# IML-DKFZ/values

Hardware: AMD Instinct MI355X
Metric: uncertainty-volumes/sec (64^3, T=10 MC-dropout) (higher is better)
Workload: dtype f32; 1 GPU; C2: 64^3 1-channel volumes, UNet3D(initial_filter_size=8, 2 classes), T=10 MC-dropout passes + fused softmax/entropy/MI/variance/argmax reduction; dropout=hash bit generator, new seed every step, weights=torch default init, seed 123

## Files before the change

### include/values_amd.h

```cpp
#ifndef VALUES_AMD_H
#define VALUES_AMD_H

#include <stddef.h>
#include <stdint.h>

#ifdef __cplusplus
extern "C" {
#endif

typedef void* vx_stream_t;

enum {
  VX_OK = 0,
  VX_E_NULL = -1,
  VX_E_SHAPE = -2,
  VX_E_DTYPE = -3,
  VX_E_WORKSPACE = -4,
  VX_E_ALIGN = -5
};

enum { VX_F32 = 0, VX_F64 = 1 };
enum { VX_ACT_NONE = 0, VX_ACT_LRELU = 1 , VX_ACT_RELU = 2 };
enum { VX_DROP_NONE = 0, VX_DROP_HASH = 1, VX_DROP_MASK = 2 };

// ... 72 lines not shown
  const int32_t* head_dst;
  const int32_t* head_flip;
  int32_t head_C;
  const float* in_mean; const float* in_rstd;
  int32_t in_drop_mode; uint32_t in_drop_seed, in_drop_layer;
  int32_t in_repeat;
  int32_t out_xblk, out_half;
  uint32_t* range_flag;
  const uint32_t* seed_dev;
  const float* up_in;
  const float* up_w;
  const float* up_b;
  int32_t up_pitch;
  float* pool_out;
  uint32_t* pool_flags;
  int32_t in_split;
  int32_t out_f16, in_f16;
  int32_t out_split, up_split;
  const float* up_fused;
  const uint32_t* in_pool_flags;
  const float* acc_in;
  int32_t acc_pitch;
  int32_t out_planar, in_planar;
  int32_t products;
} vx_conv3d_args;
int64_t vx_conv3d_upfused_packed_floats(void);
int vx_pack_conv3d_upfused(const float* w1_torch, const float* b1, const float* up_w_torch, const float* up_b, float* packed,
                           vx_stream_t stream);
int vx_conv3d_k3_prologue_ok(int D, int H, int W, int Cin, int Cout);
int vx_conv3d_k3_upfuse_ok(int D, int H, int W, int Cin, int Cout);
int64_t vx_convT_zc16_packed_floats(void);
int vx_pack_convT_zc16(const float* w_torch , float* packed, vx_stream_t stream);
int vx_conv3d_k3_skip_prologue_ok(int D, int H, int W, int Cin, int Cout, int xblk);
int vx_conv3d_k3_acc_ok(int D, int H, int W, int Cin, int Cout);
int vx_conv3d_k3_planar_ok(int D, int H, int W, int Cin, int Cout);
int vx_conv3d_k3_poolfuse_ok(int D, int H, int W, int Cin, int Cout);
int vx_conv3d_k3_presplit_ok(int D, int H, int W, int Cin, int Cout);
int vx_conv3d_k3_poolfin_ok(int Cin, int Cout);
int vx_prenorm_split(float* x, const float* mean, const float* rstd, int N, int64_t nvox, float scale, vx_stream_t stream);
int vx_pool_finish(const float* pool_raw, const uint32_t* pool_flags, const float* mean, const float* rstd, float* out,
                   int out_pitch, int N, int64_t voxels_per_sample, int drop_scale2, vx_stream_t stream);
int vx_pool_finish_z(const float* pool_raw, const uint32_t* pool_flags, const float* mean, const float* rstd, float* out,
                     int out_pitch, int N, int Dp, int64_t plane_voxels, int drop_scale2, vx_stream_t stream);
int vx_conv3d_k3_pool_layout(int D, int H, int W, int Cin, int Cout);
int vx_conv3d_k3_tiles(int D, int H, int W);
int vx_conv3d_k3_tiles_for(int D, int H, int W, int Cout);
int vx_conv3d_k3(const vx_conv3d_args* a, vx_stream_t stream);
int vx_conv3d_k3_head_fusable(int Cin, int Cout);

int vx_conv3d_k3_c1_tiles(int D, int H, int W);
int vx_conv3d_k3_c1(const float* in, const float* w_torch , const float* bias, float* out,
                    int out_pitch, int N, int D, int H, int W, int Cout, int repeat, const int32_t* src,
                    const int32_t* flip, float* stats_partial, vx_stream_t stream);

int vx_pack_input_cl8(const float* in, float* out, int N, int Cin, int D, int H, int W, int repeat, const int32_t* src,
                      const int32_t* flip, vx_stream_t stream);

int vx_instnorm_finalize(const float* stats_partial, int N, int ntiles, int C, int64_t nvox, float eps,
                         float* mean, float* rstd, vx_stream_t stream);

typedef struct vx_norm_args {
  const float* x; int32_t x_pitch;
  const float* mean; const float* rstd;
  float* out; int32_t out_pitch, out_coff;
  float* pool_out; int32_t pool_pitch;
  int32_t N, D, H, W, C;
  int32_t act, drop_mode; uint32_t drop_seed, drop_layer; const uint8_t* drop_mask;
  int32_t out_xblk, out_half;
  int32_t x_xblk, x_half;
  const uint32_t* seed_dev;
  uint32_t* range_flag;
} vx_norm_args;
int vx_norm_act_drop_pool(const vx_norm_args* a, vx_stream_t stream);
typedef struct vx_stat_src {
  const float* stats_partial; int32_t tiles; float eps; int64_t count;
  float* mean_out; float* rstd_out;
} vx_stat_src;
int vx_norm_act_drop_pool_stats(const vx_norm_args* a, const vx_stat_src* st, vx_stream_t stream);
int vx_prenorm_split_stats(float* x, const vx_stat_src* st, int N, int64_t nvox, float scale, vx_stream_t stream);
int vx_zero(void* p, int64_t bytes, vx_stream_t stream);
int vx_pool_finish_z_stats(const float* pool_raw, const uint32_t* pool_flags, const vx_stat_src* st, float* out, int out_pitch,
                           int N, int Dp, int64_t plane_voxels, int drop_scale2, vx_stream_t stream);
int vx_norm_act_drop_pool_bcast(const vx_norm_args* a, int x_repeat, vx_stream_t stream);

typedef struct vx_convT_args {
  const float* in; int32_t in_pitch;
  const float* w_packed; const float* bias;
  float* out; int32_t out_pitch, out_coff;
  int32_t N, D, H, W, Cin, Cout;
  int32_t act, drop_mode; uint32_t drop_seed, drop_layer; const uint8_t* drop_mask;
  int32_t out_xblk, out_half;
  uint32_t* range_flag;
  const uint32_t* seed_dev;
} vx_convT_args;
int vx_convT_k2s2(const vx_convT_args* a, vx_stream_t stream);

int vx_conv1x1_ncdhw(const float* in, int in_pitch, const float* w, const float* bias, float* out, int N, int D,
                     int H, int W, int F, int C, const int32_t* dst, const int32_t* flip, vx_stream_t stream);

typedef struct vx_unet3d_weights {
  const float* conv_w[18];
  const float* conv_b[18];
  const float* up_w[4];
  const float* up_b[4];
  const float* final_w;
  const float* final_b;
// ... 221 lines not shown
```

### values_amd/_lib.py

```python
from __future__ import annotations

import ctypes as C
import os

_HERE = os.path.dirname(os.path.abspath(__file__))
LIB_PATH = os.environ.get("VX_LIB_PATH") or os.path.join(_HERE, "libvalues_amd.so")

VX_F32, VX_F64 = 0, 1
VX_ACT_NONE, VX_ACT_LRELU, VX_ACT_RELU = 0, 1, 2
VX_DROP_NONE, VX_DROP_HASH, VX_DROP_MASK = 0, 1, 2

_p = C.c_void_p
_i = C.c_int
_i32 = C.c_int32
_u32 = C.c_uint32
_i64 = C.c_int64


class ConvArgs(C.Structure):
    _fields_ = [("in_", _p), ("w_packed", _p), ("bias", _p), ("out", _p),
                ("in_pitch", _i32), ("out_pitch", _i32), ("out_coff", _i32),
                ("N", _i32), ("D", _i32), ("H", _i32), ("W", _i32), ("Cin", _i32), ("Cout", _i32),
                ("act", _i32), ("drop_mode", _i32), ("drop_seed", _u32), ("drop_layer", _u32),
                ("drop_mask", _p), ("stats_partial", _p), ("in_xblk", _i32), ("w_family", _i32),
# ... 116 lines not shown
                  "distance beyond the output start", "output capacity reached", "checksum mismatch", "ISIZE mismatch",
                  "trailing bytes", "stored block length mismatch", "preset dictionary")
VX_INFLATE_CAPACITY = 7


class NiftiDecItem(C.Structure):
    _fields_ = [("src", _p), ("src_n", _i64), ("vox_offset", _i64), ("dst", _p), ("dst_n", _i64), ("ndim", _i32),
                ("dims", _i32 * 7), ("code", _i32), ("big_endian", _i32), ("out_dtype", _i32), ("pad", _i32),
                ("slope", C.c_double), ("inter", C.c_double)]


SIGNATURES = {
    "vx_version": (_i, []),
    "vx_last_error_string": (C.c_char_p, []),
    "vx_last_kernel_name": (C.c_char_p, []),
    "vx_drop_hash_mask": (_i, [_u32, _u32, _i, _i64, _p, _p]),
    "vx_get_config": (_i, [C.POINTER(Config)]),
    "vx_set_config": (_i, [C.POINTER(Config)]),
    "vx_conv3d_k3_family": (_i, [_i, _i]),
    "vx_conv2d_family": (_i, [_i, _i, _i]),
    "vx_unc_reduce": (_i, [_p, _i, _i, _i, _i, _i, _i64, _p, _p, _p, _p, _p, _p, _p]),
    "vx_unc_reduce_ex": (_i, [_p, _i, _i, _i, _i, _i, _i64, C.POINTER(UncOutputs), _p]),
    "vx_unc_stats_accumulate": (_i, [_p, _i, _i, _i, _i64, _p, _p]),
    "vx_unc_stats_finalize": (_i, [_p, _i, _i, _i, _i64, _p, _p, _p, _p, _p, _p]),
    "vx_softmax_planar": (_i, [_p, _i64, _i, _i64, _p, _p]),
    "vx_one_minus_msr": (_i, [_p, _i, _i, _i64, _p, _p]),
    "vx_conv3d_k3_packed_floats": (_i64, [_i, _i]),
    "vx_pack_conv3d_k3": (_i, [_p, _p, _i, _i, _p]),
    "vx_convT_k2s2_packed_floats": (_i64, [_i, _i]),
    "vx_pack_convT_k2s2": (_i, [_p, _p, _i, _i, _p]),
    "vx_conv3d_k3_tiles": (_i, [_i, _i, _i]),
    "vx_conv3d_k3_tiles_for": (_i, [_i, _i, _i, _i]),
    "vx_conv3d_k3_head_fusable": (_i, [_i, _i]),
    "vx_conv3d_k3_prologue_ok": (_i, [_i, _i, _i, _i, _i]),
    "vx_conv3d_k3_upfuse_ok": (_i, [_i, _i, _i, _i, _i]),
    "vx_conv3d_k3_poolfuse_ok": (_i, [_i, _i, _i, _i, _i]),
    "vx_conv3d_k3_presplit_ok": (_i, [_i, _i, _i, _i, _i]),
    "vx_conv3d_k3_poolfin_ok": (_i, [_i, _i]),
    "vx_conv3d_upfused_packed_floats": (_i64, []),
    "vx_pack_conv3d_upfused": (_i, [_p, _p, _p, _p, _p, _p]),
    "vx_pool_finish": (_i, [_p, _p, _p, _p, _p, _i, _i, _i64, _i, _p]),
    "vx_pool_finish_z": (_i, [_p, _p, _p, _p, _p, _i, _i, _i, _i64, _i, _p]),
    "vx_conv3d_k3_pool_layout": (_i, [_i, _i, _i, _i, _i]),
    "vx_conv3d_k3_skip_prologue_ok": (_i, [_i, _i, _i, _i, _i, _i]),
    "vx_conv3d_k3_acc_ok": (_i, [_i, _i, _i, _i, _i]),
    "vx_conv3d_k3_planar_ok": (_i, [_i, _i, _i, _i, _i]),
    "vx_convT_zc16_packed_floats": (_i64, []),
    "vx_pack_convT_zc16": (_i, [_p, _p, _p]),
    "vx_prenorm_split": (_i, [_p, _p, _p, _i, _i64, C.c_float, _p]),
    "vx_zero": (_i, [_p, _i64, _p]),
    "vx_conv3d_k3": (_i, [C.POINTER(ConvArgs), _p]),
    "vx_conv3d_k3_c1_tiles": (_i, [_i, _i, _i]),
    "vx_conv3d_k3_c1": (_i, [_p, _p, _p, _p, _i, _i, _i, _i, _i, _i, _i, _p, _p, _p, _p]),
    "vx_pack_input_cl8": (_i, [_p, _p, _i, _i, _i, _i, _i, _i, _p, _p, _p]),
    "vx_instnorm_finalize": (_i, [_p, _i, _i, _i, _i64, C.c_float, _p, _p, _p]),
    "vx_norm_act_drop_pool": (_i, [C.POINTER(NormArgs), _p]),
    "vx_norm_act_drop_pool_bcast": (_i, [C.POINTER(NormArgs), _i, _p]),
    "vx_norm_act_drop_pool_stats": (_i, [C.POINTER(NormArgs), C.POINTER(StatSrc), _p]),
    "vx_prenorm_split_stats": (_i, [_p, C.POINTER(StatSrc), _i, _i64, C.c_float, _p]),
    "vx_pool_finish_z_stats": (_i, [_p, _p, C.POINTER(StatSrc), _p, _i, _i, _i, _i64, _i, _p]),
    "vx_convT_k2s2": (_i, [C.POINTER(ConvTArgs), _p]),
    "vx_conv1x1_ncdhw": (_i, [_p, _i, _p, _p, _p, _i, _i, _i, _i, _i, _i, _p, _p, _p]),
    "vx_unet3d_workspace_bytes": (C.c_size_t, [_i, _i, _i, _i, _i]),
    "vx_unet3d_forward": (_i, [C.POINTER(UNet3DWeights), C.POINTER(UNet3DRun), _p]),
    "vx_unet3d_forward_profiled": (_i, [C.POINTER(UNet3DWeights), C.POINTER(UNet3DRun), _p, _i, C.POINTER(C.c_float),
                                        C.POINTER(C.c_char_p), C.POINTER(_i)]),
    "vx_softmax_accumulate": (_i, [_p, _i, _i, _i, _i, _i, _i, _p, _p, _p, _i, _i, _i, _i, _p]),
    "vx_aleatoric_sample": (_i, [_p, _p, _u32, _i, _i, _i, _i64, _p, _p, _p]),
    "vx_colorize_u8": (_i, [_p, _p, _i64, _p, _i, _p, _p]),
    "vx_fuse_sum": (_i, [C.POINTER(FuseArgs), _p]),
    "vx_tta_views_2d": (_i, [_p, _i, _p, _p, C.POINTER(C.c_float), C.POINTER(C.c_float), C.c_float, _i, _i, _i, _i,
                             C.POINTER(C.c_int32), _p, _p]),
    "vx_select_workspace_bytes": (_i64, []),
    "vx_select_kth": (_i, [_p, _i64, _i64, _p, _p, _p]),
    "vx_count_nonzero_u8": (_i, [_p, _i64, _p, _p]),
    "vx_mask_agreement": (_i, [_p, _i, _i, _i64, _p, _p]),
    "vx_soft_metric_workspace_bytes": (_i64, [_i, _i]),
    "vx_soft_metric_sums": (_i, [_p, _p, _i, _i, _i64, _p, _p, _p]),
    "vx_ssn2d_lowres": (_i, [_p, _i, _p, _i, _p, _u32, _i, _i64, _i, _i, _i, _p, _p, _p]),
    "vx_ssn2d_add_diag": (_i, [_p, _p, _p, _u32, _i, _i, _i64, C.c_float, _p]),
    "vx_softmax_variance": (_i, [_p, _i, _i, _i, _i, _i64, _p, _p]),
    "vx_ssn_sample": (_i, [_p, _p, _p, _u32, _i, _i, _i, _i, _i64, C.c_float, _p, _p]),
    "vx_conv2d_packed_floats": (_i64, [_i, _i, _i]),
    "vx_pack_conv2d": (_i, [_p, _p, _i, _i, _i, _p]),
    "vx_conv2d_tiles": (_i, [_i, _i, _i, _i]),
    "vx_conv2d": (_i, [C.POINTER(Conv2dArgs), _p]),
    "vx_bn_finalize": (_i, [_p, _i, _i, _i64, C.c_float, _p, _p, _p, _p, _p]),
    "vx_bn_finalize_groups": (_i, [_p, _i, _i, _i, _i, _i64, C.c_float, _p, _p, _p, _p, _p]),
    "vx_affine_gather": (_i, [C.POINTER(AffineArgs), _p]),
    "vx_bilinear_nchw": (_i, [_p, _i, _i, _i, _i, _i, _i, _i, _p, _p, _p, _p]),
    "vx_bilinear_softmax_nchw": (_i, [_p, _i, _i, _i, _i, _i, _i, _i, _p, _p, _p, _p]),
    "vx_evalmetrics_workspace_bytes": (_i64, []),
    "vx_ncc_sums": (_i, [_p, _i, _p, _i, _i64, _i, C.c_double, C.c_double, _p, _p, _p]),
    "vx_platt_sums": (_i, [_p, _i, _p, _p, _i, _i64, _i, C.c_double, C.c_double, C.c_double, C.c_double, _p, _p, _p]),
    "vx_calib_bins": (_i, [_p, _i, _p, _p, _i, _i64, _i, C.c_double, C.c_double, C.POINTER(C.c_double), _p, _p, _p]),
    "vx_box_max": (_i, [_p, _i, _i, _i, _i, _i, _i, _p, _p, _p, C.c_size_t, _p]),
    "vx_sum_thr": (_i, [_p, _i, _i64, C.c_double, _p, _p]),
    "vx_nifti_workspace_bytes": (C.c_size_t, [_i]),
    "vx_nifti_payload_bytes": (_i64, [C.POINTER(NiftiItem)]),
    "vx_nifti_payload": (_i, [C.POINTER(NiftiItem), _i, _p, _i64, _p, C.c_size_t, _p]),
    "vx_gzip_bound": (_i64, [_i64]),
    "vx_gzip_workspace_bytes": (C.c_size_t, [C.POINTER(_i64), _i]),
    "vx_gzip_encode": (_i, [C.POINTER(GzItem), _i, _p, _i64, _p, _p, C.c_size_t, _p]),
    "vx_crc32": (_i, [_p, _i64, _p, _p]),
    "vx_png_bound": (_i64, [_i, _i]),
    "vx_png_workspace_bytes": (C.c_size_t, [C.POINTER(PngItem), _i]),
# ... 91 lines not shown
```

### values_amd/csrc/conv3d_c1.hip

```cpp
#include "s16_common.h"

template <int COUT>
__global__ __launch_bounds__(256) void conv3d_k3_c1_kernel(const float* __restrict__ in, const float* __restrict__ w,
                                                           const float* __restrict__ bias,
                                                           float* __restrict__ out, int out_pitch, int N, int D, int H, int W,
                                                           int repeat, const int32_t* __restrict__ src,
                                                           const int32_t* __restrict__ flip, float* __restrict__ stats_partial,
                                                           int tiles_x, int tiles_y, int tiles_z) {
  constexpr int TX = 64, TY = 4, TZ = 4;
  constexpr int HX = TX + 2, HY = TY + 2, HZ = TZ + 2;
  __shared__ float s_in[HZ * HY * HX];
  __shared__ __attribute__((aligned(16))) float s_w[27 * COUT];
  __shared__ float s_red[16][COUT][2];

  const int tid = threadIdx.x;
  int t = blockIdx.x;
  const int tx = t % tiles_x; t /= tiles_x;
  const int ty = t % tiles_y; t /= tiles_y;
  const int tz = t % tiles_z; t /= tiles_z;
  const int n = t;
  const int v = src ? src[n] : n / repeat;
  const int f = flip ? flip[n] : 0;
  const int x0 = tx * TX, y0 = ty * TY, z0 = tz * TZ;
  const float* in_v = in + (size_t)v * D * H * W;

  for (int idx = tid; idx < HZ * HY * HX; idx += 256) {
    const int hx = idx % HX, hy = (idx / HX) % HY, hz = idx / (HX * HY);
    int gx = x0 + hx - 1, gy = y0 + hy - 1, gz = z0 + hz - 1;
    float val = 0.f;
    if ((unsigned)gx < (unsigned)W && (unsigned)gy < (unsigned)H && (unsigned)gz < (unsigned)D) {
      if (f & 1) gz = D - 1 - gz;
      if (f & 2) gy = H - 1 - gy;
      if (f & 4) gx = W - 1 - gx;
      val = in_v[((size_t)gz * H + gy) * W + gx];
    }
    s_in[idx] = val;
  }
  for (int idx = tid; idx < 27 * COUT; idx += 256) {
    const int co = idx % COUT, tap = idx / COUT;
    s_w[idx] = w[co * 27 + tap];
  }
  __syncthreads();

  const int lx = tid % TX, ly = tid / TX;
  float acc[TZ][COUT];
#pragma unroll
  for (int z = 0; z < TZ; ++z)
#pragma unroll
    for (int c = 0; c < COUT; ++c) acc[z][c] = bias[c];
#pragma unroll 1
  for (int kk = 0; kk < 9; ++kk) {
    const int ky = kk / 3, kx = kk - 3 * ky;
    float wk[3][COUT];
#pragma unroll
    for (int kz = 0; kz < 3; ++kz)
#pragma unroll
      for (int c = 0; c < COUT; c += 4) {
        const f32x4 w4 = *reinterpret_cast<const f32x4*>(&s_w[(kz * 9 + kk) * COUT + c]);
        wk[kz][c] = w4[0]; wk[kz][c + 1] = w4[1]; wk[kz][c + 2] = w4[2]; wk[kz][c + 3] = w4[3];
      }
    const float* sp = s_in + (ly + ky) * HX + lx + kx;
#pragma unroll
    for (int p = 0; p < HZ; ++p) {
      const float xv = sp[p * HY * HX];
#pragma unroll
      for (int z = 0; z < TZ; ++z) {
        const int kz = p - z;
        if (kz < 0 || kz > 2) continue;
#pragma unroll
        for (int c = 0; c < COUT; ++c) acc[z][c] = fmaf(wk[kz][c], xv, acc[z][c]);
      }
    }
  }

  const int gx = x0 + lx, gy = y0 + ly;
  float ssum[COUT], ssq[COUT];
#pragma unroll
  for (int c = 0; c < COUT; ++c) { ssum[c] = 0.f; ssq[c] = 0.f; }
#pragma unroll
  for (int z = 0; z < TZ; ++z) {
    const int gz = z0 + z;
    const bool valid = gx < W && gy < H && gz < D;
    if (valid) {
      float* o = out + (((size_t)(n * D + gz) * H + gy) * W + gx) * out_pitch;
#pragma unroll
      for (int c = 0; c < COUT; c += 4)
        *reinterpret_cast<f32x4*>(o + c) = (f32x4){acc[z][c], acc[z][c + 1], acc[z][c + 2], acc[z][c + 3]};
#pragma unroll
      for (int c = 0; c < COUT; ++c) { ssum[c] += acc[z][c]; ssq[c] = fmaf(acc[z][c], acc[z][c], ssq[c]); }
    }
  }
  if (stats_partial) {
    const int lane = tid & 63, wave = tid >> 6;
#pragma unroll
    for (int c = 0; c < COUT; ++c) {
      float s = ssum[c], q = ssq[c];
#pragma unroll
      for (int rot = 8; rot >= 1; rot >>= 1) { s += vx_row_ror(s, rot); q += vx_row_ror(q, rot); }
      if ((lane & 15) == 0) { s_red[wave * 4 + (lane >> 4)][c][0] = s; s_red[wave * 4 + (lane >> 4)][c][1] = q; }
    }
    __syncthreads();
    if (tid < COUT) {
      float s = 0.f, q = 0.f;
#pragma unroll
      for (int wv = 0; wv < 16; ++wv) { s += s_red[wv][tid][0]; q += s_red[wv][tid][1]; }
      const int ntiles = tiles_x * tiles_y * tiles_z;
      const int tile = blockIdx.x % ntiles;
      float* dst = stats_partial + (((size_t)n * ntiles + tile) * COUT + tid) * 2;
      dst[0] = s;
      dst[1] = q;
    }
  }
}

extern "C" int vx_conv3d_k3_c1_tiles(int D, int H, int W) { return ((W + 63) / 64) * ((H + 3) / 4) * ((D + 3) / 4); }

extern "C" int vx_conv3d_k3_c1(const float* in, const float* w_torch, const float* bias, float* out, int out_pitch,
                               int N, int D, int H, int W, int Cout, int repeat, const int32_t* src,
                               const int32_t* flip, float* stats_partial, vx_stream_t stream) {
  if (!in || !w_torch || !bias || !out) VX_FAIL(VX_E_NULL, "vx_conv3d_k3_c1: null pointer");
  if (N <= 0 || D <= 0 || H <= 0 || W <= 0) VX_FAIL(VX_E_SHAPE, "vx_conv3d_k3_c1: empty tensor");
  if (repeat <= 0) VX_FAIL(VX_E_SHAPE, "vx_conv3d_k3_c1: repeat must be >= 1");
  if (out_pitch < Cout || out_pitch % 4 || !vx_aligned16(out)) VX_FAIL(VX_E_ALIGN, "vx_conv3d_k3_c1: out pitch/alignment");
  const int tiles_x = (W + 63) / 64, tiles_y = (H + 3) / 4, tiles_z = (D + 3) / 4;
  dim3 grid((unsigned)(tiles_x * tiles_y * tiles_z * N));
  hipStream_t s = (hipStream_t)stream;
#define VX_C1(CO)                                                                                                  \
  vx_note_kernel("conv3d_k3_c1_kernel<" #CO ">");                                                                  \
  hipLaunchKernelGGL(conv3d_k3_c1_kernel<CO>, grid, dim3(256), 0, s, in, w_torch, bias, out, out_pitch, N, D, H, W, \
                     repeat, src, flip, stats_partial, tiles_x, tiles_y, tiles_z)
  switch (Cout) {
    case 8: VX_C1(8); break;
    case 16: VX_C1(16); break;
    case 32: VX_C1(32); break;
    default: VX_FAIL(VX_E_SHAPE, "vx_conv3d_k3_c1: Cout=%d unsupported (8, 16, 32)", Cout);
  }
#undef VX_C1
  VX_CHECK_LAUNCH("vx_conv3d_k3_c1");
  return VX_OK;
}

__global__ __launch_bounds__(256) void pack_input_cl8_kernel(const float* __restrict__ in, float* __restrict__ out, int N, int Cin,
                                                             int D, int H, int W, int repeat, const int32_t* __restrict__ src,
                                                             const int32_t* __restrict__ flip) {
  const int64_t nvox = (int64_t)D * H * W, total = (int64_t)N * nvox;
  for (int64_t i = blockIdx.x * (int64_t)blockDim.x + threadIdx.x; i < total; i += (int64_t)gridDim.x * blockDim.x) {
    const int n = (int)(i / nvox);
    const int64_t v = i - (int64_t)n * nvox;
    int x = (int)(v % W), y = (int)((v / W) % H), z = (int)(v / ((int64_t)W * H));
    const int vol = src ? src[n] : n / repeat;
    const int fl = flip ? flip[n] : 0;
    if (fl & 1) z = D - 1 - z;
    if (fl & 2) y = H - 1 - y;
    if (fl & 4) x = W - 1 - x;
    const float* p = in + ((size_t)vol * Cin) * nvox + ((size_t)z * H + y) * W + x;
    f32x4 lo = {0.f, 0.f, 0.f, 0.f}, hi = {0.f, 0.f, 0.f, 0.f};
#pragma unroll
    for (int c = 0; c < 4; ++c) {
      if (c < Cin) lo[c] = p[(size_t)c * nvox];
      if (c + 4 < Cin) hi[c] = p[(size_t)(c + 4) * nvox];
    }
    reinterpret_cast<f32x4*>(out + (size_t)i * 8)[0] = lo;
    reinterpret_cast<f32x4*>(out + (size_t)i * 8)[1] = hi;
  }
}

extern "C" int vx_pack_input_cl8(const float* in, float* out, int N, int Cin, int D, int H, int W, int repeat,
                                 const int32_t* src, const int32_t* flip, vx_stream_t stream) {
  if (!in || !out) VX_FAIL(VX_E_NULL, "vx_pack_input_cl8: null pointer");
  if (N <= 0 || D <= 0 || H <= 0 || W <= 0 || repeat <= 0) VX_FAIL(VX_E_SHAPE, "vx_pack_input_cl8: empty tensor");
  if (Cin < 1 || Cin > 8) VX_FAIL(VX_E_SHAPE, "vx_pack_input_cl8: in_channels %d (1 .. 8)", Cin);
  if (!vx_aligned16(out)) VX_FAIL(VX_E_ALIGN, "vx_pack_input_cl8: output alignment");
  const int64_t total = (int64_t)N * D * H * W;
  int bx = (int)((total + 255) / 256);
  if (bx > 16384) bx = 16384;
  vx_note_kernel("pack_input_cl8_kernel");
  hipLaunchKernelGGL(pack_input_cl8_kernel, dim3(bx), dim3(256), 0, (hipStream_t)stream, in, out, N, Cin, D, H, W, repeat, src, flip);
  VX_CHECK_LAUNCH("vx_pack_input_cl8");
  return VX_OK;
}
```

### values_amd/csrc/lib.cpp

```cpp
#include <stdarg.h>
#include <stdio.h>
#include <stdlib.h>
#include <string.h>

#include "../../include/values_amd.h"

static thread_local char g_err[512] = "";

void vx_set_error(const char* fmt, ...) {
  va_list ap;
  va_start(ap, fmt);
  vsnprintf(g_err, sizeof(g_err), fmt, ap);
  va_end(ap);
}

static thread_local const char* g_last_kernel = nullptr;
void vx_note_kernel(const char* name) { g_last_kernel = name; }
const char* vx_last_kernel() { return g_last_kernel; }
const char* vx_kname(const char* fmt, ...) {
  char buf[256];
  va_list ap;
  va_start(ap, fmt);
  vsnprintf(buf, sizeof(buf), fmt, ap);
  va_end(ap);
// ... 6 lines not shown
#include <stdlib.h>
#include <string.h>

static vx_config g_cfg;
static std::once_flag g_cfg_once;

static int env_int(const char* name, int dflt) {
  const char* e = getenv(name);
  if (!e || !*e) return dflt;
  char* end = nullptr;
  const long v = strtol(e, &end, 0);
  return end == e ? 1 : (int)v;
}

static void cfg_from_env() {
  memset(&g_cfg, 0, sizeof(g_cfg));
  g_cfg.conv_fp32 = env_int("VX_CONV_FP32", 0);
  g_cfg.s16_no_prenorm = env_int("VX_S16_NO_PRENORM", 0);
  g_cfg.s16_no_xp8 = env_int("VX_S16_NO_XP8", 0);
  g_cfg.s16_skip_raw = env_int("VX_S16_SKIP_RAW", 1);
  g_cfg.no_head_fusion = env_int("VX_NO_HEAD_FUSION", 0);
  g_cfg.s16_no_upfuse = env_int("VX_S16_NO_UPFUSE", 0);
  g_cfg.s16_no_poolfuse = env_int("VX_S16_NO_POOLFUSE", 0);
  g_cfg.storage16 = env_int("VX_STORAGE16", 0);
  g_cfg.s16_generic = env_int("VX_S16_GENERIC", 0);
  g_cfg.s16_no_zc16 = env_int("VX_S16_NO_ZC16", 0);
  g_cfg.s16_no_halves = env_int("VX_S16_NO_HALVES", 0);
  g_cfg.s16_no_deep = env_int("VX_S16_NO_DEEP", 0);
  g_cfg.s16_no_l1dma = env_int("VX_S16_NO_L1DMA", 0);
  g_cfg.c2s_no_wide = env_int("VX_C2S_NO_WIDE", 0);
  g_cfg.c2s_no_oct = env_int("VX_C2S_NO_OCT", 0);
}

const vx_config& vx_cfg() {
  std::call_once(g_cfg_once, cfg_from_env);
  return g_cfg;
}

extern "C" int vx_get_config(vx_config* out) {
  if (!out) { vx_set_error("vx_get_config: null"); return VX_E_NULL; }
  *out = vx_cfg();
  return VX_OK;
}

extern "C" int vx_set_config(const vx_config* cfg) {
  if (!cfg) { vx_set_error("vx_set_config: null"); return VX_E_NULL; }
  if (cfg->conv_fp32 < 0 || cfg->conv_fp32 > 2) { vx_set_error("vx_set_config: conv_fp32 %d", cfg->conv_fp32); return VX_E_DTYPE; }
  (void)vx_cfg();
  g_cfg = *cfg;
  return VX_OK;
}

extern "C" const char* vx_last_kernel_name(void) { return g_last_kernel ? g_last_kernel : ""; }
extern "C" int vx_version(void) { return 720;  }
extern "C" const char* vx_last_error_string(void) { return g_err; }
```

### values_amd/csrc/unet3d_forward.hip

```cpp
#include "common.h"
#include <stdlib.h>

extern "C" int vx_conv3d_k3_c1_tiles(int D, int H, int W);

namespace {
struct Level { int D, H, W, C; int64_t nvox; };

struct Plan {
  Level lv[5];
  float *A[4], *B[4], *CAT[4], *P[5], *C0, *C1;
  float *stats, *mean, *rstd;
  float *mean0, *rstd0;
  float *meanS[4], *rstdS[4];
  size_t bytes;
};

static size_t align_up(size_t v) { return (v + 255) & ~(size_t)255; }

static void make_plan(Plan& p, int N, int D, int H, int W, int F, char* base) {
  size_t off = 0;
  auto carve = [&](size_t floats) {
    float* q = base ? (float*)(base + off) : nullptr;
    off += align_up(floats * sizeof(float));
    return q;
  };
  for (int l = 0; l < 5; ++l) {
    p.lv[l].D = D >> l; p.lv[l].H = H >> l; p.lv[l].W = W >> l; p.lv[l].C = F << l;
    p.lv[l].nvox = (int64_t)p.lv[l].D * p.lv[l].H * p.lv[l].W;
  }
  for (int l = 0; l < 4; ++l) {
    const size_t e = (size_t)N * p.lv[l].nvox * p.lv[l].C;
    p.A[l] = carve(e);
    p.B[l] = carve(e);
    p.CAT[l] = carve(2 * e);
  }
  p.P[0] = nullptr;
  for (int l = 1; l < 5; ++l) p.P[l] = carve((size_t)N * p.lv[l].nvox * p.lv[l - 1].C);
  p.C0 = carve((size_t)N * p.lv[4].nvox * p.lv[4].C);
  p.C1 = carve((size_t)N * p.lv[4].nvox * p.lv[4].C);
  size_t smax = 0;
  for (int l = 0; l < 4; ++l) {
    size_t t = (size_t)vx_conv3d_k3_tiles(p.lv[l].D, p.lv[l].H, p.lv[l].W);
    if (l == 0) {
      size_t t1 = (size_t)vx_conv3d_k3_c1_tiles(p.lv[0].D, p.lv[0].H, p.lv[0].W);
      if (t1 > t) t = t1;
    }
    const size_t e = (size_t)N * t * p.lv[l].C * 2;
    if (e > smax) smax = e;
  }
  p.stats = carve(smax);
  p.mean = carve((size_t)N * p.lv[3].C);
  p.rstd = carve((size_t)N * p.lv[3].C);
  p.mean0 = carve((size_t)N * p.lv[0].C);
  p.rstd0 = carve((size_t)N * p.lv[0].C);
  for (int l = 0; l < 4; ++l) {
    p.meanS[l] = l == 0 ? p.mean0 : carve((size_t)N * p.lv[l].C);
// ... 3 lines not shown
}
}

extern "C" size_t vx_unet3d_workspace_bytes(int N, int D, int H, int W, int F) {
  if (N <= 0 || D <= 0 || H <= 0 || W <= 0 || F <= 0) return 0;
  Plan p;
  make_plan(p, N, D, H, W, F, nullptr);
  return p.bytes;
}

namespace {
struct Prof {
  static constexpr int MAXL = 96;
  hipEvent_t ev[2 * MAXL];
  const char* name[MAXL];
  const char* kernel[MAXL];
  int n = 0;
  hipStream_t s;
};
thread_local Prof* g_prof = nullptr;
thread_local char g_prof_labels[Prof::MAXL][192];
}

#define VX_TRY(expr)            \
  do {                          \
    int rc_ = (expr);           \
    if (rc_ != VX_OK) return rc_; \
  } while (0)

#define VX_STEP(label, expr)                                                       \
  do {                                                                             \
    Prof* pf_ = g_prof;                                                            \
    if (pf_ && pf_->n < Prof::MAXL) { vx_note_kernel(nullptr); (void)hipEventRecord(pf_->ev[2 * pf_->n], pf_->s); }  \
    int rc_ = (expr);                                                              \
    if (rc_ != VX_OK) return rc_;                                                  \
    if (pf_ && pf_->n < Prof::MAXL) {                                              \
      (void)hipEventRecord(pf_->ev[2 * pf_->n + 1], pf_->s);                             \
      pf_->kernel[pf_->n] = vx_last_kernel();                                      \
      pf_->name[pf_->n++] = (label);                                               \
    }                                                                              \
  } while (0)

namespace {
int xblk_of(int W) { return W % 4 == 0 ? 4 : (W % 2 == 0 ? 2 : 1); }

struct Flow {
  bool inorm;
  int ich;
  int rep;
  bool shared;
  bool fuse_head;
  bool pre[4];
  bool presplit;
  bool skip_raw[4];
  bool pooled[4];
  bool poolfin1;
  bool halves[4];
  bool fuse_up;
  bool fuse_up1;
  bool split_out[4];
  bool planar1;
  bool st16;
  int products_c12, products_e11, products_e12;
};

Flow decide_flow(const vx_unet3d_weights* w, const vx_unet3d_run* r, const Plan& p) {
  const vx_config& cfg = vx_cfg();
  const int F = w->F, dm = r->drop_mode;
  const Level* lv = p.lv;
  const bool hashed = dm != VX_DROP_MASK;
  Flow f = {};
  f.inorm = !w->no_instancenorm;
  f.ich = w->in_channels > 1 ? w->in_channels : 1;
  f.rep = r->repeat > 0 ? r->repeat : 1;
  f.shared = !r->src && !r->flip && f.rep > 1 && r->N % f.rep == 0;
  f.fuse_head = w->num_classes <= 4 && vx_conv3d_k3_head_fusable(F, F) && !cfg.no_head_fusion;
  f.pre[0] = hashed && !cfg.s16_no_prenorm && F == 8 && f.inorm && vx_conv3d_k3_prologue_ok(lv[0].D, lv[0].H, lv[0].W, F, F);
  for (int l = 1; l < 4; ++l)
    f.pre[l] = f.inorm && hashed && !cfg.s16_no_prenorm && vx_conv3d_k3_prologue_ok(lv[l].D, lv[l].H, lv[l].W, lv[l].C, lv[l].C);
  f.presplit = f.shared && f.pre[0] && vx_conv3d_k3_presplit_ok(lv[0].D, lv[0].H, lv[0].W, F, F);
  f.skip_raw[0] = f.pre[0] && cfg.s16_skip_raw && vx_conv3d_k3_prologue_ok(lv[0].D, lv[0].H, lv[0].W, 2 * F, F);
  f.pooled[0] = f.skip_raw[0] && vx_conv3d_k3_poolfuse_ok(lv[0].D, lv[0].H, lv[0].W, F, F);
  f.poolfin1 = f.pooled[0] && vx_conv3d_k3_poolfin_ok(F, 2 * F);
  for (int l = 1; l < 4; ++l) {
    const Level& L = lv[l];
    f.skip_raw[l] = f.pooled[l] = f.inorm && hashed && !cfg.s16_no_prenorm && cfg.s16_skip_raw &&
                                  vx_conv3d_k3_pool_layout(L.D, L.H, L.W, L.C, L.C) == 2 &&
                                  vx_conv3d_k3_skip_prologue_ok(L.D, L.H, L.W, 2 * L.C, L.C, xblk_of(L.W));
  }
  f.halves[1] = f.skip_raw[1] && lv[1].C == 16 && w->split_w[0] && w->split_w[1] && !cfg.s16_no_halves &&
                w->split_family == vx_conv3d_k3_family(16, 16) && vx_conv3d_k3_acc_ok(lv[1].D, lv[1].H, lv[1].W, 16, 16);
  f.fuse_up = hashed && F == 8 && vx_conv3d_k3_upfuse_ok(lv[0].D, lv[0].H, lv[0].W, 2 * F, F);
  f.fuse_up1 = f.halves[1] && w->up3_zc16 && hashed && vx_conv3d_k3_upfuse_ok(lv[1].D, lv[1].H, lv[1].W, 16, 16) == 2;
  f.split_out[1] = f.fuse_up;
  f.split_out[2] = f.fuse_up1;
  f.planar1 = f.fuse_up1 && !cfg.s16_no_l1dma && vx_conv3d_k3_planar_ok(lv[1].D, lv[1].H, lv[1].W, 16, 16);
  f.st16 = cfg.storage16 && dm == VX_DROP_HASH && F == 8 && f.fuse_head && cfg.conv_fp32 == 0 &&
           vx_conv3d_k3_prologue_ok(lv[0].D, lv[0].H, lv[0].W, F, F);
  const bool one = f.st16 && cfg.storage16 == 2;
  f.products_c12 = one && f.presplit && f.pooled[0];
  f.products_e11 = one && f.skip_raw[0] && f.fuse_up && w->up_fused;
  f.products_e12 = one;
  return f;
}
}

extern "C" int vx_unet3d_forward(const vx_unet3d_weights* w, const vx_unet3d_run* r, vx_stream_t stream) {
  if (!w || !r) VX_FAIL(VX_E_NULL, "vx_unet3d_forward: null argument");
  if (!r->x || !r->logits || !r->workspace) VX_FAIL(VX_E_NULL, "vx_unet3d_forward: null tensor/workspace");
  const int N = r->N, D = r->D, H = r->H, W = r->W, F = w->F, NC = w->num_classes;
  if (N <= 0 || D <= 0 || H <= 0 || W <= 0) VX_FAIL(VX_E_SHAPE, "vx_unet3d_forward: empty batch");
  if (D % 16 || H % 16 || W % 16)
    VX_FAIL(VX_E_SHAPE, "vx_unet3d_forward: spatial size (%d,%d,%d) must be divisible by 16 (4 poolings; InstanceNorm "
            "needs > 1 voxel at the 8x level)", D, H, W);
  if (F != 8 && F != 16 && F != 32) VX_FAIL(VX_E_SHAPE, "vx_unet3d_forward: initial_filter_size %d unsupported (8,16,32)", F);
  if (NC <= 0) VX_FAIL(VX_E_SHAPE, "vx_unet3d_forward: num_classes %d", NC);
  if (r->drop_mode < 0 || r->drop_mode > 2) VX_FAIL(VX_E_DTYPE, "vx_unet3d_forward: drop_mode %d", r->drop_mode);
  if ((((uintptr_t)r->workspace) & 255u) != 0) VX_FAIL(VX_E_ALIGN, "vx_unet3d_forward: workspace must be 256-byte aligned");
  for (int i = 0; i < 18; ++i)
    if (!w->conv_w[i] || !w->conv_b[i]) VX_FAIL(VX_E_NULL, "vx_unet3d_forward: conv weight %d missing", i);
  if (w->in_channels < 0 || w->in_channels > 8) VX_FAIL(VX_E_SHAPE, "vx_unet3d_forward: in_channels %d (1 .. 8)", w->in_channels);
  for (int i = 0; i < 4; ++i)
    if (!w->up_w[i] || !w->up_b[i]) VX_FAIL(VX_E_NULL, "vx_unet3d_forward: transposed-conv weight %d missing", i);
  if (!w->final_w || !w->final_b) VX_FAIL(VX_E_NULL, "vx_unet3d_forward: final weights missing");
  if (r->drop_mode == VX_DROP_MASK)
    for (int i = 0; i < 17; ++i)
      if (!r->masks[i]) VX_FAIL(VX_E_NULL, "vx_unet3d_forward: mask %d missing", i);

  Plan p;
  make_plan(p, N, D, H, W, F, (char*)r->workspace);
  if (p.bytes > r->workspace_bytes)
    VX_FAIL(VX_E_WORKSPACE, "vx_unet3d_forward: workspace %zu B < required %zu B", r->workspace_bytes, p.bytes);
  const Flow f = decide_flow(w, r, p);

  const int dm = r->drop_mode;
  auto mask = [&](int i) { return dm == VX_DROP_MASK ? r->masks[i] : (const uint8_t*)nullptr; };
  auto conv_args = [&](int wi, const Level& L, int Cin, int Cout, float* stats) {
    vx_conv3d_args a = {};
    a.w_packed = w->conv_w[wi]; a.bias = w->conv_b[wi]; a.w_family = w->conv_family[wi];
// ... 19 lines not shown
    a.act = VX_ACT_LRELU;
    a.drop_mode = drop_layer >= 0 ? dm : VX_DROP_NONE; a.drop_seed = r->seed; a.drop_layer = (uint32_t)(drop_layer >= 0 ? drop_layer : 0);
    a.drop_mask = drop_layer >= 0 ? mask(drop_layer) : nullptr;
    a.seed_dev = r->seed_dev;
    return a;
  };
  auto convT = [&](const float* in, int ui, float* out, int out_pitch, const Level& Lin, int Cin, int Cout, int act,
                   int drop_layer, bool dense) {
    vx_convT_args a = {};
    a.range_flag = r->range_flag;
    a.seed_dev = r->seed_dev;
    a.out_xblk = dense ? 0 : xblk_of(2 * Lin.W); a.out_half = 0;
    a.in = in; a.in_pitch = Cin; a.w_packed = w->up_w[ui]; a.bias = w->up_b[ui];
    a.out = out; a.out_pitch = out_pitch; a.out_coff = 0;
    a.N = N; a.D = Lin.D; a.H = Lin.H; a.W = Lin.W; a.Cin = Cin; a.Cout = Cout;
    a.act = act;
    a.drop_mode = drop_layer >= 0 ? dm : VX_DROP_NONE;
    a.drop_seed = r->seed; a.drop_layer = (uint32_t)(drop_layer >= 0 ? drop_layer : 0);
    a.drop_mask = drop_layer >= 0 ? mask(drop_layer) : nullptr;
    return vx_convT_k2s2(&a, stream);
  };
  auto pool_flags = [&](int l) {
    const size_t maxima = l == 0 ? (size_t)N * p.lv[1].nvox * 8 : (size_t)N * (p.lv[l].nvox / 4) * p.lv[l].C;
    return reinterpret_cast<uint32_t*>(p.B[l] + maxima);
  };
  auto first_conv = [&](float* out, int n_out, int rep, float* stats) -> int {
    const Level& L = p.lv[0];
    if (f.ich == 1)
      return vx_conv3d_k3_c1(r->x, w->conv_w[0], w->conv_b[0], out, L.C, n_out, L.D, L.H, L.W, L.C, rep, r->src, r->flip, stats, stream);
    VX_TRY(vx_pack_input_cl8(r->x, p.B[0], n_out, f.ich, L.D, L.H, L.W, rep, r->src, r->flip, stream));
    vx_conv3d_args a = conv_args(0, L, 8, L.C, stats);
    a.N = n_out; a.in = p.B[0]; a.in_pitch = 8; a.out = out; a.out_pitch = L.C;
    return vx_conv3d_k3(&a, stream);
  };

  static const char* kConv[18] = {"contr_1_1", "contr_1_2", "contr_2_1", "contr_2_2", "contr_3_1", "contr_3_2",
                                  "contr_4_1", "contr_4_2", "center.0", "center.2", "expand_4_1", "expand_4_2",
                                  "expand_3_1", "expand_3_2", "expand_2_1", "expand_2_2", "expand_1_1", "expand_1_2"};
  static const char* kNorm[8] = {"norm:contr_1_1", "norm:contr_1_2", "norm:contr_2_1", "norm:contr_2_2",
                                 "norm:contr_3_1", "norm:contr_3_2", "norm:contr_4_1", "norm:contr_4_2"};
  static const char* kFin[8] = {"finalize:contr_1_1", "finalize:contr_1_2", "finalize:contr_2_1", "finalize:contr_2_2",
                                "finalize:contr_3_1", "finalize:contr_3_2", "finalize:contr_4_1", "finalize:contr_4_2"};
  static const char* kPoolFin[4] = {"poolfin:contr_1_2", "poolfin:contr_2_2", "poolfin:contr_3_2", "poolfin:contr_4_2"};
  static const char* kUp[4] = {"center.4", "upscale4", "upscale3", "upscale2"};
  float* const out1 = f.shared && !f.skip_raw[0] ? p.CAT[0] : p.A[0];
  const int fan = f.shared ? f.rep : 1;
  for (int l = 0; l < 4; ++l) {
    const Level& L = p.lv[l];
    const int C = L.C;
    const int ntiles = vx_conv3d_k3_tiles_for(L.D, L.H, L.W, C);
    if (l == 0) {
      const int n1 = N / fan;
      const int ntiles1 = f.ich == 1 ? vx_conv3d_k3_c1_tiles(L.D, L.H, L.W) : ntiles;
      VX_STEP(kConv[0], first_conv(out1, n1, f.shared ? 1 : f.rep, f.inorm ? p.stats : nullptr));
      if (f.inorm) VX_STEP(kFin[0], vx_instnorm_finalize(p.stats, n1, ntiles1, C, L.nvox, 1e-5f, p.mean, p.rstd, stream));
      if (f.presplit)
        VX_STEP("presplit:contr_1_1", vx_prenorm_split(out1, p.mean, p.rstd, n1, L.nvox, dm == VX_DROP_HASH ? 2.f : 1.f, stream));
      if (!f.pre[0]) {
        vx_norm_args n = norm_args(out1, C, L, 0, f.inorm);
        n.out = p.A[0]; n.out_pitch = C;
        VX_STEP(kNorm[0], vx_norm_act_drop_pool_bcast(&n, fan, stream));
      }
    } else {
      vx_conv3d_args a = conv_args(2 * l, L, C / 2, C, f.inorm ? p.stats : nullptr);
      a.in = p.P[l]; a.in_pitch = C / 2; a.out = p.A[l]; a.out_pitch = C;
      if (!f.inorm) set_drop(a, VX_ACT_LRELU, 2 * l);
      if (l == 1 && f.poolfin1) {
        a.in = p.B[0]; a.in_pool_flags = pool_flags(0);
        set_pre(a, 1, 1, p.mean0, p.rstd0);
      }
      VX_STEP(l == 1 && f.poolfin1 ? "poolfin+contr_2_1" : kConv[2 * l], vx_conv3d_k3(&a, stream));
      if (f.inorm) {
        VX_STEP(kFin[2 * l], vx_instnorm_finalize(p.stats, N, ntiles, C, L.nvox, 1e-5f, p.mean, p.rstd, stream));
        if (!f.pre[l]) {
          vx_norm_args n = norm_args(p.A[l], C, L, 2 * l, true);
          n.out = p.A[l]; n.out_pitch = C;
          VX_STEP(kNorm[2 * l], vx_norm_act_drop_pool_bcast(&n, 1, stream));
        }
      }
    }
    if (!f.inorm) {
      vx_conv3d_args a = conv_args(2 * l + 1, L, C, C, nullptr);
      a.in = p.A[l]; a.in_pitch = C; a.out = p.B[l]; a.out_pitch = C;
      set_drop(a, VX_ACT_LRELU, 2 * l + 1);
      VX_STEP(kConv[2 * l + 1], vx_conv3d_k3(&a, stream));
      vx_norm_args n = norm_args(p.B[l], C, L, -1, false);
      n.act = VX_ACT_NONE;
      n.out = p.CAT[l]; n.out_pitch = 2 * C; n.out_coff = C; n.out_xblk = xblk_of(L.W); n.pool_out = p.P[l + 1];
      VX_STEP(kNorm[2 * l + 1], vx_norm_act_drop_pool_bcast(&n, 1, stream));
      continue;
    }
    vx_conv3d_args a = conv_args(2 * l + 1, L, C, C, p.stats);
    a.in = p.A[l]; a.in_pitch = C; a.out = p.B[l]; a.out_pitch = C;
    if (f.pre[l]) {
      if (l == 0) a.in = out1;
      set_pre(a, 2 * l, l == 0 ? fan : 1, p.mean, p.rstd);
    }
    a.in_split = l == 0 && f.presplit;
    if (l == 0) a.products = f.products_c12;
    if (f.skip_raw[l]) {
      if (f.halves[l]) a.out = p.CAT[l] + (size_t)N * L.nvox * C;
      else { a.out = p.CAT[l]; a.out_xblk = xblk_of(L.W); }
    }
    if (f.pooled[l]) {
      a.pool_out = p.B[l]; a.pool_flags = pool_flags(l);
      set_drop(a, VX_ACT_NONE, 2 * l + 1);
    }
    VX_STEP(kConv[2 * l + 1], vx_conv3d_k3(&a, stream));
    if (l == 0 && f.skip_raw[0]) {
// ... 121 lines not shown
```

Baseline: 3897 volumes/s.

## Recompute first Cin=1 conv twice to fuse stats and prenorm split

The first 1-channel conv now runs twice: a stats-only pass that skips writing raw output, and a second pass that recomputes the conv and applies the instance-norm, leaky ReLU, dropout scale and fp16 hi/lo split directly before storing. This drops the raw fp32 write plus the separate prenorm_split read/write pass, trading bandwidth for duplicate cheap arithmetic on one input channel. The halo load is also restructured so each wave loads whole rows, with the edge columns handled separately.

```diff
diff --git a/include/values_amd.h b/include/values_amd.h
--- a/include/values_amd.h
+++ b/include/values_amd.h
@@ -148,6 +148,11 @@
 int vx_conv3d_k3_c1(const float* in, const float* w_torch , const float* bias, float* out,
                     int out_pitch, int N, int D, int H, int W, int Cout, int repeat, const int32_t* src,
                     const int32_t* flip, float* stats_partial, vx_stream_t stream);
+int vx_conv3d_k3_c1_stats(const float* in, const float* w_torch, const float* bias, int N, int D, int H, int W, int Cout,
+                          int repeat, const int32_t* src, const int32_t* flip, float* stats_partial, vx_stream_t stream);
+int vx_conv3d_k3_c1_split(const float* in, const float* w_torch, const float* bias, const float* mean, const float* rstd,
+                          float scale, float* out, int N, int D, int H, int W, int Cout, int repeat, const int32_t* src,
+                          const int32_t* flip, vx_stream_t stream);
 
 int vx_pack_input_cl8(const float* in, float* out, int N, int Cin, int D, int H, int W, int repeat, const int32_t* src,
                       const int32_t* flip, vx_stream_t stream);
diff --git a/values_amd/_lib.py b/values_amd/_lib.py
--- a/values_amd/_lib.py
+++ b/values_amd/_lib.py
@@ -192,6 +192,8 @@
     "vx_conv3d_k3": (_i, [C.POINTER(ConvArgs), _p]),
     "vx_conv3d_k3_c1_tiles": (_i, [_i, _i, _i]),
     "vx_conv3d_k3_c1": (_i, [_p, _p, _p, _p, _i, _i, _i, _i, _i, _i, _i, _p, _p, _p, _p]),
+    "vx_conv3d_k3_c1_stats": (_i, [_p, _p, _p, _i, _i, _i, _i, _i, _i, _p, _p, _p, _p]),
+    "vx_conv3d_k3_c1_split": (_i, [_p, _p, _p, _p, _p, C.c_float, _p, _i, _i, _i, _i, _i, _i, _p, _p, _p]),
     "vx_pack_input_cl8": (_i, [_p, _p, _i, _i, _i, _i, _i, _i, _p, _p, _p]),
     "vx_instnorm_finalize": (_i, [_p, _i, _i, _i, _i64, C.c_float, _p, _p, _p]),
     "vx_norm_act_drop_pool": (_i, [C.POINTER(NormArgs), _p]),
diff --git a/values_amd/csrc/conv3d_c1.hip b/values_amd/csrc/conv3d_c1.hip
--- a/values_amd/csrc/conv3d_c1.hip
+++ b/values_amd/csrc/conv3d_c1.hip
@@ -1,12 +1,16 @@
 #include "s16_common.h"
 
-template <int COUT>
+enum { C1_RAW = 0, C1_STATS = 1, C1_SPLIT = 2 };
+
+template <int COUT, int MODE>
 __global__ __launch_bounds__(256) void conv3d_k3_c1_kernel(const float* __restrict__ in, const float* __restrict__ w,
                                                            const float* __restrict__ bias,
                                                            float* __restrict__ out, int out_pitch, int N, int D, int H, int W,
                                                            int repeat, const int32_t* __restrict__ src,
                                                            const int32_t* __restrict__ flip, float* __restrict__ stats_partial,
-                                                           int tiles_x, int tiles_y, int tiles_z) {
+                                                           int tiles_x, int tiles_y, int tiles_z,
+                                                           const float* __restrict__ mean, const float* __restrict__ rstd, float scale) {
+  static_assert(MODE != C1_SPLIT || COUT == 8, "the pre-split layout is that of an 8-channel tensor");
   constexpr int TX = 64, TY = 4, TZ = 4;
   constexpr int HX = TX + 2, HY = TY + 2, HZ = TZ + 2;
   __shared__ float s_in[HZ * HY * HX];
@@ -24,8 +28,8 @@
   const int x0 = tx * TX, y0 = ty * TY, z0 = tz * TZ;
   const float* in_v = in + (size_t)v * D * H * W;
 
-  for (int idx = tid; idx < HZ * HY * HX; idx += 256) {
-    const int hx = idx % HX, hy = (idx / HX) % HY, hz = idx / (HX * HY);
+  auto halo = [&](int row, int hx) {
+    const int hz = row / HY, hy = row - hz * HY;
     int gx = x0 + hx - 1, gy = y0 + hy - 1, gz = z0 + hz - 1;
     float val = 0.f;
     if ((unsigned)gx < (unsigned)W && (unsigned)gy < (unsigned)H && (unsigned)gz < (unsigned)D) {
@@ -34,8 +38,13 @@
       if (f & 4) gx = W - 1 - gx;
       val = in_v[((size_t)gz * H + gy) * W + gx];
     }
-    s_in[idx] = val;
-  }
+    s_in[row * HX + hx] = val;
+  };
+  static_assert(HZ * HY % 4 == 0 && 2 * HZ * HY <= 256, "rows per wave / edge columns");
+  const int wv = __builtin_amdgcn_readfirstlane(tid >> 6);
+#pragma unroll
+  for (int k = 0; k < HZ * HY / 4; ++k) halo(wv + 4 * k, (tid & 63) + 1);
+  if (tid < 2 * HZ * HY) halo(tid >> 1, (tid & 1) ? HX - 1 : 0);
   for (int idx = tid; idx < 27 * COUT; idx += 256) {
     const int co = idx % COUT, tap = idx / COUT;
     s_w[idx] = w[co * 27 + tap];
@@ -74,6 +83,36 @@
   }
 
   const int gx = x0 + lx, gy = y0 + ly;
+  if constexpr (MODE == C1_SPLIT) {
+    float mu[COUT], sc[COUT];
+#pragma unroll
+    for (int c = 0; c < COUT; ++c) { mu[c] = mean[(size_t)n * COUT + c]; sc[c] = rstd[(size_t)n * COUT + c] * scale; }
+#pragma unroll
+    for (int z = 0; z < TZ; ++z) {
+      const int gz = z0 + z;
+      if (gx < W && gy < H && gz < D) {
+        float* o = out + (((size_t)(n * D + gz) * H + gy) * W + gx) * COUT;
+#pragma unroll
+        for (int c = 0; c < COUT; c += 4) {
+          f32x4 v;
+#pragma unroll
+          for (int j = 0; j < 4; ++j) {
+            const float t = (acc[z][c + j] - mu[c + j]) * sc[c + j];
+            v[j] = fmaxf(t, 0.01f * t);
+          }
+          f16x4 hi, lo;
+          vx_split4(v, hi, lo);
+          f32x4 p;
+          p[0] = __builtin_bit_cast(float, (f16x2){hi[0], hi[1]});
+          p[1] = __builtin_bit_cast(float, (f16x2){hi[2], hi[3]});
+          p[2] = __builtin_bit_cast(float, (f16x2){lo[0], lo[1]});
+          p[3] = __builtin_bit_cast(float, (f16x2){lo[2], lo[3]});
+          *reinterpret_cast<f32x4*>(o + c) = p;
+        }
+      }
+    }
+    return;
+  }
   float ssum[COUT], ssq[COUT];
 #pragma unroll
   for (int c = 0; c < COUT; ++c) { ssum[c] = 0.f; ssq[c] = 0.f; }
@@ -82,10 +121,12 @@
     const int gz = z0 + z;
     const bool valid = gx < W && gy < H && gz < D;
     if (valid) {
-      float* o = out + (((size_t)(n * D + gz) * H + gy) * W + gx) * out_pitch;
-#pragma unroll
-      for (int c = 0; c < COUT; c += 4)
-        *reinterpret_cast<f32x4*>(o + c) = (f32x4){acc[z][c], acc[z][c + 1], acc[z][c + 2], acc[z][c + 3]};
+      if constexpr (MODE == C1_RAW) {
+        float* o = out + (((size_t)(n * D + gz) * H + gy) * W + gx) * out_pitch;
+#pragma unroll
+        for (int c = 0; c < COUT; c += 4)
+          *reinterpret_cast<f32x4*>(o + c) = (f32x4){acc[z][c], acc[z][c + 1], acc[z][c + 2], acc[z][c + 3]};
+      }
 #pragma unroll
       for (int c = 0; c < COUT; ++c) { ssum[c] += acc[z][c]; ssq[c] = fmaf(acc[z][c], acc[z][c], ssq[c]); }
     }
@@ -115,29 +156,60 @@
 
 extern "C" int vx_conv3d_k3_c1_tiles(int D, int H, int W) { return ((W + 63) / 64) * ((H + 3) / 4) * ((D + 3) / 4); }
 
+namespace {
+int c1_launch(int mode, const char* who, const float* in, const float* w_torch, const float* bias, float* out, int out_pitch, int N,
+              int D, int H, int W, int Cout, int repeat, const int32_t* src, const int32_t* flip, float* stats_partial,
+              const float* mean, const float* rstd, float scale, vx_stream_t stream) {
+  if (!in || !w_torch || !bias) VX_FAIL(VX_E_NULL, "%s: null pointer", who);
+  if (N <= 0 || D <= 0 || H <= 0 || W <= 0) VX_FAIL(VX_E_SHAPE, "%s: empty tensor", who);
+  if (repeat <= 0) VX_FAIL(VX_E_SHAPE, "%s: repeat must be >= 1", who);
+  const int tiles_x = (W + 63) / 64, tiles_y = (H + 3) / 4, tiles_z = (D + 3) / 4;
+  dim3 grid((unsigned)(tiles_x * tiles_y * tiles_z * N));
+  hipStream_t s = (hipStream_t)stream;
+#define VX_C1(CO, MODE)                                                                                                  \
+  vx_note_kernel("conv3d_k3_c1_kernel<" #CO "," #MODE ">");                                                              \
+  hipLaunchKernelGGL((conv3d_k3_c1_kernel<CO, MODE>), grid, dim3(256), 0, s, in, w_torch, bias, out, out_pitch, N, D, H, W, \
+                     repeat, src, flip, stats_partial, tiles_x, tiles_y, tiles_z, mean, rstd, scale)
+  if (mode == C1_RAW) {
+    switch (Cout) {
+      case 8: VX_C1(8, 0); break;
+      case 16: VX_C1(16, 0); break;
+      case 32: VX_C1(32, 0); break;
+      default: VX_FAIL(VX_E_SHAPE, "%s: Cout=%d unsupported (8, 16, 32)", who, Cout);
+    }
+  } else {
+    if (Cout != 8) VX_FAIL(VX_E_SHAPE, "%s: Cout=%d unsupported (8)", who, Cout);
+    if (mode == C1_STATS) { VX_C1(8, 1); } else { VX_C1(8, 2); }
+  }
+#undef VX_C1
+  VX_CHECK_LAUNCH(who);
+  return VX_OK;
+}
+}
+
 extern "C" int vx_conv3d_k3_c1(const float* in, const float* w_torch, const float* bias, float* out, int out_pitch,
                                int N, int D, int H, int W, int Cout, int repeat, const int32_t* src,
                                const int32_t* flip, float* stats_partial, vx_stream_t stream) {
-  if (!in || !w_torch || !bias || !out) VX_FAIL(VX_E_NULL, "vx_conv3d_k3_c1: null pointer");
-  if (N <= 0 || D <= 0 || H <= 0 || W <= 0) VX_FAIL(VX_E_SHAPE, "vx_conv3d_k3_c1: empty tensor");
-  if (repeat <= 0) VX_FAIL(VX_E_SHAPE, "vx_conv3d_k3_c1: repeat must be >= 1");
+  if (!out) VX_FAIL(VX_E_NULL, "vx_conv3d_k3_c1: null pointer");
   if (out_pitch < Cout || out_pitch % 4 || !vx_aligned16(out)) VX_FAIL(VX_E_ALIGN, "vx_conv3d_k3_c1: out pitch/alignment");
-  const int tiles_x = (W + 63) / 64, tiles_y = (H + 3) / 4, tiles_z = (D + 3) / 4;
-  dim3 grid((unsigned)(tiles_x * tiles_y * tiles_z * N));
-  hipStream_t s = (hipStream_t)stream;
-#define VX_C1(CO)                                                                                                  \
-  vx_note_kernel("conv3d_k3_c1_kernel<" #CO ">");                                                                  \
-  hipLaunchKernelGGL(conv3d_k3_c1_kernel<CO>, grid, dim3(256), 0, s, in, w_torch, bias, out, out_pitch, N, D, H, W, \
-                     repeat, src, flip, stats_partial, tiles_x, tiles_y, tiles_z)
-  switch (Cout) {
-    case 8: VX_C1(8); break;
-    case 16: VX_C1(16); break;
-    case 32: VX_C1(32); break;
-    default: VX_FAIL(VX_E_SHAPE, "vx_conv3d_k3_c1: Cout=%d unsupported (8, 16, 32)", Cout);
-  }
-#undef VX_C1
-  VX_CHECK_LAUNCH("vx_conv3d_k3_c1");
-  return VX_OK;
+  return c1_launch(C1_RAW, "vx_conv3d_k3_c1", in, w_torch, bias, out, out_pitch, N, D, H, W, Cout, repeat, src, flip, stats_partial,
+                   nullptr, nullptr, 1.f, stream);
+}
+
+extern "C" int vx_conv3d_k3_c1_stats(const float* in, const float* w_torch, const float* bias, int N, int D, int H, int W, int Cout,
+                                     int repeat, const int32_t* src, const int32_t* flip, float* stats_partial, vx_stream_t stream) {
+  if (!stats_partial) VX_FAIL(VX_E_NULL, "vx_conv3d_k3_c1_stats: null pointer");
+  return c1_launch(C1_STATS, "vx_conv3d_k3_c1_stats", in, w_torch, bias, nullptr, 0, N, D, H, W, Cout, repeat, src, flip, stats_partial,
+                   nullptr, nullptr, 1.f, stream);
+}
+
+extern "C" int vx_conv3d_k3_c1_split(const float* in, const float* w_torch, const float* bias, const float* mean, const float* rstd,
+                                     float scale, float* out, int N, int D, int H, int W, int Cout, int repeat, const int32_t* src,
+                                     const int32_t* flip, vx_stream_t stream) {
+  if (!out || !mean || !rstd) VX_FAIL(VX_E_NULL, "vx_conv3d_k3_c1_split: null pointer");
+  if (!vx_aligned16(out)) VX_FAIL(VX_E_ALIGN, "vx_conv3d_k3_c1_split: out alignment");
+  return c1_launch(C1_SPLIT, "vx_conv3d_k3_c1_split", in, w_torch, bias, out, 8, N, D, H, W, Cout, repeat, src, flip, nullptr,
+                   mean, rstd, scale, stream);
 }
 
 __global__ __launch_bounds__(256) void pack_input_cl8_kernel(const float* __restrict__ in, float* __restrict__ out, int N, int Cin,
diff --git a/values_amd/csrc/lib.cpp b/values_amd/csrc/lib.cpp
--- a/values_amd/csrc/lib.cpp
+++ b/values_amd/csrc/lib.cpp
@@ -82,5 +82,5 @@
 }
 
 extern "C" const char* vx_last_kernel_name(void) { return g_last_kernel ? g_last_kernel : ""; }
-extern "C" int vx_version(void) { return 720;  }
+extern "C" int vx_version(void) { return 730;  }
 extern "C" const char* vx_last_error_string(void) { return g_err; }
diff --git a/values_amd/csrc/unet3d_forward.hip b/values_amd/csrc/unet3d_forward.hip
--- a/values_amd/csrc/unet3d_forward.hip
+++ b/values_amd/csrc/unet3d_forward.hip
@@ -2,6 +2,11 @@
 #include <stdlib.h>
 
 extern "C" int vx_conv3d_k3_c1_tiles(int D, int H, int W);
+extern "C" int vx_conv3d_k3_c1_stats(const float* in, const float* w_torch, const float* bias, int N, int D, int H, int W, int Cout,
+                                     int repeat, const int32_t* src, const int32_t* flip, float* stats_partial, vx_stream_t stream);
+extern "C" int vx_conv3d_k3_c1_split(const float* in, const float* w_torch, const float* bias, const float* mean, const float* rstd,
+                                     float scale, float* out, int N, int D, int H, int W, int Cout, int repeat, const int32_t* src,
+                                     const int32_t* flip, vx_stream_t stream);
 
 namespace {
 struct Level { int D, H, W, C; int64_t nvox; };
@@ -111,6 +116,7 @@
   bool fuse_head;
   bool pre[4];
   bool presplit;
+  bool c1_twice;
   bool skip_raw[4];
   bool pooled[4];
   bool poolfin1;
@@ -129,21 +135,23 @@
   const Level* lv = p.lv;
   const bool hashed = dm != VX_DROP_MASK;
   Flow f = {};
+  const bool prenorm = cfg.s16_no_prenorm != 1;
   f.inorm = !w->no_instancenorm;
   f.ich = w->in_channels > 1 ? w->in_channels : 1;
   f.rep = r->repeat > 0 ? r->repeat : 1;
   f.shared = !r->src && !r->flip && f.rep > 1 && r->N % f.rep == 0;
   f.fuse_head = w->num_classes <= 4 && vx_conv3d_k3_head_fusable(F, F) && !cfg.no_head_fusion;
-  f.pre[0] = hashed && !cfg.s16_no_prenorm && F == 8 && f.inorm && vx_conv3d_k3_prologue_ok(lv[0].D, lv[0].H, lv[0].W, F, F);
+  f.pre[0] = hashed && prenorm && F == 8 && f.inorm && vx_conv3d_k3_prologue_ok(lv[0].D, lv[0].H, lv[0].W, F, F);
   for (int l = 1; l < 4; ++l)
-    f.pre[l] = f.inorm && hashed && !cfg.s16_no_prenorm && vx_conv3d_k3_prologue_ok(lv[l].D, lv[l].H, lv[l].W, lv[l].C, lv[l].C);
+    f.pre[l] = f.inorm && hashed && prenorm && vx_conv3d_k3_prologue_ok(lv[l].D, lv[l].H, lv[l].W, lv[l].C, lv[l].C);
   f.presplit = f.shared && f.pre[0] && vx_conv3d_k3_presplit_ok(lv[0].D, lv[0].H, lv[0].W, F, F);
+  f.c1_twice = f.presplit && f.ich == 1 && cfg.s16_no_prenorm != 2;
   f.skip_raw[0] = f.pre[0] && cfg.s16_skip_raw && vx_conv3d_k3_prologue_ok(lv[0].D, lv[0].H, lv[0].W, 2 * F, F);
   f.pooled[0] = f.skip_raw[0] && vx_conv3d_k3_poolfuse_ok(lv[0].D, lv[0].H, lv[0].W, F, F);
   f.poolfin1 = f.pooled[0] && vx_conv3d_k3_poolfin_ok(F, 2 * F);
   for (int l = 1; l < 4; ++l) {
     const Level& L = lv[l];
-    f.skip_raw[l] = f.pooled[l] = f.inorm && hashed && !cfg.s16_no_prenorm && cfg.s16_skip_raw &&
+    f.skip_raw[l] = f.pooled[l] = f.inorm && hashed && prenorm && cfg.s16_skip_raw &&
                                   vx_conv3d_k3_pool_layout(L.D, L.H, L.W, L.C, L.C) == 2 &&
                                   vx_conv3d_k3_skip_prologue_ok(L.D, L.H, L.W, 2 * L.C, L.C, xblk_of(L.W));
   }
@@ -269,9 +277,15 @@
     if (l == 0) {
       const int n1 = N / fan;
       const int ntiles1 = f.ich == 1 ? vx_conv3d_k3_c1_tiles(L.D, L.H, L.W) : ntiles;
-      VX_STEP(kConv[0], first_conv(out1, n1, f.shared ? 1 : f.rep, f.inorm ? p.stats : nullptr));
+      if (f.c1_twice)
+        VX_STEP("stats:contr_1_1", vx_conv3d_k3_c1_stats(r->x, w->conv_w[0], w->conv_b[0], n1, L.D, L.H, L.W, C, 1, nullptr, nullptr, p.stats, stream));
+      else
+        VX_STEP(kConv[0], first_conv(out1, n1, f.shared ? 1 : f.rep, f.inorm ? p.stats : nullptr));
       if (f.inorm) VX_STEP(kFin[0], vx_instnorm_finalize(p.stats, n1, ntiles1, C, L.nvox, 1e-5f, p.mean, p.rstd, stream));
-      if (f.presplit)
+      if (f.c1_twice)
+        VX_STEP(kConv[0], vx_conv3d_k3_c1_split(r->x, w->conv_w[0], w->conv_b[0], p.mean, p.rstd, dm == VX_DROP_HASH ? 2.f : 1.f, out1, n1,
+                                                L.D, L.H, L.W, C, 1, nullptr, nullptr, stream));
+      else if (f.presplit)
         VX_STEP("presplit:contr_1_1", vx_prenorm_split(out1, p.mean, p.rstd, n1, L.nvox, dm == VX_DROP_HASH ? 2.f : 1.f, stream));
       if (!f.pre[0]) {
         vx_norm_args n = norm_args(out1, C, L, 0, f.inorm);
```

Result: no change. 3910 volumes/s (median of 6 runs) (+0.3%).
